# risc-mi/totalsegmentator2D

Measured on AMD Instinct MI355X. Metric: 2-ch 512x512 slices/sec, higher is better.
Workload: dtype f32 storage/accumulate, products as 3x fp16-split MFMA (f16x3)

## Files before the change

totalsegmentator2d_amd/_lib.py:

```python
from __future__ import annotations

import ctypes
import os

_HERE = os.path.dirname(os.path.abspath(__file__))
LIB_PATH = os.path.join(_HERE, 'libts2d_engine.so')
HEADER_PATH = os.path.join(os.path.dirname(_HERE), 'include', 'ts2d_engine.h')
ABI_VERSION = 9
MAX_STAGES = 16
PRECISION_F32_EXACT = 0
PRECISION_F32_SPLIT_F16X3 = 1
PRECISION_F16 = 2

class ArchDesc(ctypes.Structure):
    _fields_ = [('input_channels', ctypes.c_int32), ('num_classes', ctypes.c_int32), ('n_stages', ctypes.c_int32),
                ('features', ctypes.c_int32 * MAX_STAGES), ('n_conv_enc', ctypes.c_int32 * MAX_STAGES),
                ('n_conv_dec', ctypes.c_int32 * MAX_STAGES), ('norm_eps', ctypes.c_float), ('leaky_slope', ctypes.c_float),
                ('strides', (ctypes.c_int32 * 2) * MAX_STAGES)]


class ResidualDesc(ctypes.Structure):
    _fields_ = [('n_blocks', ctypes.c_int32 * MAX_STAGES), ('reserved', ctypes.c_int32 * 16)]


class TiledImage(ctypes.Structure):
    _fields_ = [('image', ctypes.c_void_p), ('Hp', ctypes.c_int32), ('Wp', ctypes.c_int32), ('n_tiles', ctypes.c_int32),
                ('tile_y', ctypes.c_void_p), ('tile_x', ctypes.c_void_p), ('logits_f16', ctypes.c_void_p), ('seg_u8', ctypes.c_void_p),
                ('inf_flag', ctypes.c_int32)]


class TiledExport(ctypes.Structure):
    _fields_ = [('src_y', ctypes.c_int32), ('src_x', ctypes.c_int32), ('src_h', ctypes.c_int32), ('src_w', ctypes.c_int32),
                ('out_h', ctypes.c_int32), ('out_w', ctypes.c_int32), ('seg_u8', ctypes.c_void_p), ('logits_f32', ctypes.c_void_p)]


class TiledLabelmap(ctypes.Structure):
    _fields_ = [('src_y', ctypes.c_int32), ('src_x', ctypes.c_int32), ('src_h', ctypes.c_int32), ('src_w', ctypes.c_int32),
                ('out_h', ctypes.c_int32), ('out_w', ctypes.c_int32), ('label_u8', ctypes.c_void_p)]


class TiledProbabilities(ctypes.Structure):
    _fields_ = [('src_y', ctypes.c_int32), ('src_x', ctypes.c_int32), ('src_h', ctypes.c_int32), ('src_w', ctypes.c_int32),
                ('out_h', ctypes.c_int32), ('out_w', ctypes.c_int32), ('full_h', ctypes.c_int32), ('full_w', ctypes.c_int32),
                ('box_y', ctypes.c_int32), ('box_x', ctypes.c_int32), ('prob_f32', ctypes.c_void_p), ('decided_u8', ctypes.c_void_p)]


PROB_MULTILABEL, PROB_LABELMAP, PROB_REGIONS = 0, 1, 2

_I, _P, _Z, _LL, _ULL, _S = ctypes.c_int, ctypes.c_void_p, ctypes.c_size_t, ctypes.c_longlong, ctypes.c_ulonglong, ctypes.c_char_p
_PP, _TI, _TE, _TL = ctypes.POINTER(_P), ctypes.POINTER(TiledImage), ctypes.POINTER(TiledExport), ctypes.POINTER(TiledLabelmap)
_TP = ctypes.POINTER(TiledProbabilities)
_PROJECT = [_I, _P, _Z, _I, _I, _I, _I, _LL, _LL, _LL, _LL, _P, _P]

SIGNATURES = {
    'ts2d_abi_version': (_I, []),
    'ts2d_last_error': (_S, []),
    'ts2d_engine_create': (_I, [ctypes.POINTER(ArchDesc), _P, _Z, _I, _PP]),
    'ts2d_engine_create_residual': (_I, [ctypes.POINTER(ArchDesc), ctypes.POINTER(ResidualDesc), _P, _Z, _I, _PP]),
    'ts2d_engine_load_weights': (_I, [_P, _P, _Z]),
# ... 9 lines not shown
    'ts2d_labelmap_from_logits': (_I, [_I, _P, _I, _I, _I, ctypes.POINTER(ctypes.c_int32 * 4), _I, _I, _P]),
    'ts2d_ensemble_predict_tiled_regions': (_I, [_PP, _I, _TI, _TL, _I, _I, _I, _I, _P, _I, _P, _I]),
    'ts2d_regions_from_logits': (_I, [_I, _P, _I, _I, _I, ctypes.POINTER(ctypes.c_int32 * 4), _I, _I, _P, _P]),
    'ts2d_ensemble_predict_tiled_probabilities': (_I, [_PP, _I, _TI, _TP, _I, _I, _I, _I, _P, _I, _I, _P, _I]),
    'ts2d_probabilities_from_logits': (_I, [_I, _P, _I, _I, _I, ctypes.POINTER(ctypes.c_int32 * 4), _I, _I, _I, _I, _I, _I, _I, _P, _P, _P]),
    'ts2d_project_coronal': (_I, _PROJECT),
    'ts2d_project_coronal_zscore': (_I, _PROJECT + [_P, _P, _P]),
    'ts2d_resample_cubic': (_I, [_I, _P, _I, _I, _I, _I, _I, _P, _P]),
    'ts2d_planes_create': (_I, [_I, _P, _I, _I, _I, _PP]),
    'ts2d_planes_crop_zscore': (_I, [_P, ctypes.POINTER(ctypes.c_int32 * 4), _P, ctypes.POINTER(_I)]),
    'ts2d_planes_crop_normalize': (_I, [_P, _P, _P, _P, ctypes.POINTER(ctypes.c_int32 * 4), _P, ctypes.POINTER(_I)]),
    'ts2d_planes_create_stack': (_I, [_I, _P, _I, _I, _I, _I, _PP]),
    'ts2d_planes_crop_normalize_stack': (_I, [_P, _P, _P, _P, ctypes.POINTER(ctypes.c_int32 * 6), _P, ctypes.POINTER(_I)]),
    'ts2d_planes_resample_cubic': (_I, [_P, _I, _I]),
    'ts2d_planes_extent': (_I, [_P, ctypes.POINTER(_I), ctypes.POINTER(_I)]),
    'ts2d_planes_download': (_I, [_P, _P]),
    'ts2d_planes_destroy': (_I, [_P]),
    'ts2d_synth_slices': (_I, [_I, _ULL, _ULL, _ULL, _P, _P]),
    'ts2d_engine_reserve': (_I, [_P, _I, _I, _I]),
    'ts2d_engine_workspace_bytes': (_I, [_P, _I, _I, _I, ctypes.POINTER(_Z)]),
    'ts2d_engine_set_workspace': (_I, [_P, _P, _Z]),
    'ts2d_engine_set_precision': (_I, [_P, _I]),
    'ts2d_engine_set_option': (_I, [_P, _S, _I]),
    'ts2d_engine_set_tile_dtype': (_I, [_P, _I]),
    'ts2d_engine_set_keep_activations': (_I, [_P, _I]),
    'ts2d_engine_set_profiling': (_I, [_P, _I]),
    'ts2d_engine_num_ops': (_I, [_P]),
    'ts2d_engine_op_name': (_S, [_P, _I]),
    'ts2d_engine_op_kernel': (_S, [_P, _I]),
    'ts2d_engine_op_ksplit': (_I, [_P, _I]),
    'ts2d_engine_op_times': (_I, [_P, _P, _I]),
    'ts2d_engine_debug_tensor': (_I, [_P, _S, _P, _Z, ctypes.POINTER(ctypes.c_int32 * 4)]),
    'ts2d_engine_tiled_inf_flag': (_I, [_P]),
    'ts2d_engine_device_bytes': (_Z, [_P]),
    'ts2d_engine_destroy': (_I, [_P]),
}
SYMBOLS = tuple(SIGNATURES)
OPTIONAL = frozenset(n for n in SIGNATURES if n == 'ts2d_resample_cubic' or n.startswith('ts2d_planes_') or 'probabilities' in n or n == 'ts2d_engine_create_residual')


class EngineLibraryError(RuntimeError):
    pass


_lib = None


def build(verbose: bool = False) -> str:
    import subprocess
    subprocess.check_call(['make', '-C', os.path.join(_HERE, 'csrc')] + ([] if verbose else ['-s']))
    return LIB_PATH


def load():
    global _lib
    if _lib is not None:
        return _lib
    if not os.path.exists(LIB_PATH):
        raise EngineLibraryError(
            f"{LIB_PATH} is missing: the MI355X HIP engine has not been built (run `python -c 'import "
            f"__graft_entry__ as g; g.build()'` or `make -C totalsegmentator2d_amd/csrc`). There is no CPU fallback.")
    try:
        lib = ctypes.CDLL(LIB_PATH)
    except OSError as ex:
        raise EngineLibraryError(f"failed to load {LIB_PATH}: {ex}") from ex
    for name, (restype, argtypes) in SIGNATURES.items():
        if name in OPTIONAL and not hasattr(lib, name):
            continue
        fn = getattr(lib, name)
        fn.restype, fn.argtypes = restype, list(argtypes)
        if name == 'ts2d_abi_version' and fn() != ABI_VERSION:
            raise EngineLibraryError(f"ABI mismatch: library {fn()}, binding {ABI_VERSION}")
    _lib = lib
    return lib


def load_cffi():
    try:
        import cffi
    except ImportError:
        return None
    import re
    ffi = cffi.FFI()
    src = open(HEADER_PATH).read()
    src = re.sub(r'/\*.*?\*/', '', src, flags=re.S)
    src = '\n'.join(l for l in src.splitlines() if not l.strip().startswith('#') and 'extern "C"' not in l
                    and l.strip() not in ('}',))
    src = src.replace('TS2D_MAX_STAGES', str(MAX_STAGES))
    ffi.cdef(src)
    return ffi, ffi.dlopen(LIB_PATH)


def last_error() -> str:
    return load().ts2d_last_error().decode('utf-8', 'replace')


def check(rc: int, what: str):
    if rc != 0:
        raise RuntimeError(f"{what} failed ({rc}): {last_error()}")
```

totalsegmentator2d_amd/csrc/engine.hip:

```cpp
#include "engine_internal.h"
#include "kernels.h"
#include "kernels_f16x3.h"
#include "kernels_f16x3_convt.h"
#include "kernels_h32.h"
#include "kernels_head.h"
#include "kernels_f16x3_one.h"
#include "kernels_f16x3_qp.h"
#include "kernels_first.h"
#include "kernels_res32.h"
#include "kernels_s2v2.h"
#include "kernels_upc.h"
#include "kernels_up0.h"
#include "kernels_upq.h"
#include "kernels_upc_h.h"
#include "kernels_upc_h2.h"
#include "kernels_resblock.h"

#include <atomic>
#include <cstdio>
#include <cmath>
#include <cstdlib>
#include <cstring>
#include <string>
#include <type_traits>
// ... 611 lines not shown
    TRY(workspace_acquire(e, st));
    if (e->ws_external) {
        e->ws_token = ++g_ws_generation;
        if (!e->ws_token) e->ws_token = ++g_ws_generation;
        HIP_TRY(hipMemsetD32Async(reinterpret_cast<hipDeviceptr_t>(e->d_ws), (int)e->ws_token, 1, st));
    }
    if (clear_flags) HIP_TRY(hipMemsetAsync(e->d_flags, 0, 2 * sizeof(int), st));
    const int rc = run_forward_impl(e, d_in, B, H, W, d_logits, d_mask, st, full);
    const int rc2 = workspace_release(e, st);
    return rc != TS2D_OK ? rc : rc2;
}

int ts2d::reserve_checked(ts2d_engine* e, int B, int H, int W, bool full) {
    const int divy = 1 << e->lvl_y[e->arch.n_stages - 1], divx = 1 << e->lvl_x[e->arch.n_stages - 1];
    if (B < 1 || H < divy || W < divx || H % divy || W % divx)
        return fail(TS2D_ERR_INVALID, "shape B=%d H=%d W=%d: H and W must be positive multiples of %d and %d", B, H, W, divy, divx);
    if ((H / divy) * (W / divx) <= 1)
        return fail(TS2D_ERR_INVALID, "shape %dx%d leaves a single bottleneck pixel: InstanceNorm needs more than 1 spatial element", H, W);
    if ((long long)B * H * W >= (1LL << 31)) return fail(TS2D_ERR_INVALID, "B*H*W = %lld exceeds 2^31 pixels per call", (long long)B * H * W);
    return ensure_workspace(e, B, H, W, full);
}

extern "C" {

int ts2d_abi_version(void) { return 9; }

const char* ts2d_last_error(void) { return last_error(); }

static int create_engine(const char* entry, const ts2d_arch_desc* arch, const ts2d_residual_desc* res, const float* weights, size_t n_floats, int device,
                         ts2d_engine** out) {
    if (!arch || !out) return fail(TS2D_ERR_INVALID, "%s: null argument", entry);
    *out = nullptr;
    if (res) for (int v : res->reserved) if (v) return fail(TS2D_ERR_INVALID, "%s: ts2d_residual_desc.reserved must be zero", entry);
    int ndev = 0;
    HIP_TRY(hipGetDeviceCount(&ndev));
    if (device < 0 || device >= ndev) return fail(TS2D_ERR_INVALID, "device %d out of range (%d HIP devices visible)", device, ndev);
    ts2d_engine* e = new (std::nothrow) ts2d_engine();
    if (!e) return fail(TS2D_ERR_NOMEM, "host allocation failed");
    e->user_arch = *arch; e->device = device;
    if (res) { e->residual = true; for (int s = 0; s < TS2D_MAX_STAGES; ++s) e->n_blocks[s] = res->n_blocks[s]; }
    if (arch->n_stages >= 2 && arch->n_stages <= TS2D_MAX_STAGES) e->arch = pad_arch(*arch, e->padded); else e->arch = *arch;
    {
        hipDeviceProp_t prop;
        if (hipGetDeviceProperties(&prop, device) == hipSuccess && prop.multiProcessorCount > 0) e->num_cus = prop.multiProcessorCount;
        if (getenv("TS2D_DBG")) e->dbg = atoi(getenv("TS2D_DBG"));
    }
    int rc = build_program(e);
    if (rc != TS2D_OK) { delete e; return rc; }
    hipError_t he = hipSetDevice(device);
    if (he == hipSuccess) he = hipStreamCreateWithFlags(&e->stream, hipStreamNonBlocking);
    if (he == hipSuccess) he = hipEventCreateWithFlags(&e->ws_event, hipEventDisableTiming);
    if (he == hipSuccess) he = hipMalloc(reinterpret_cast<void**>(&e->d_flags), 2 * sizeof(int));
    if (he == hipSuccess) he = hipMemset(e->d_flags, 0, 2 * sizeof(int));
    if (he == hipSuccess && e->dbg == 256) he = hipMalloc(reinterpret_cast<void**>(&e->d_prof), 512 * 128 * sizeof(unsigned long long));
    if (he == hipSuccess && e->d_prof) he = hipMemset(e->d_prof, 0, 512 * 128 * sizeof(unsigned long long));
    if (he == hipSuccess) he = hipMalloc(reinterpret_cast<void**>(&e->d_weights), e->weight_floats * sizeof(float));
    if (he != hipSuccess) {
        rc = fail(he == hipErrorOutOfMemory ? TS2D_ERR_NOMEM : TS2D_ERR_HIP, "engine setup failed: %s", hipGetErrorString(he));
        ts2d_engine_destroy(e);
        return rc;
    }
    if (weights) {
        rc = upload_weights(e, weights, n_floats);
        if (rc != TS2D_OK) { ts2d_engine_destroy(e); return rc; }
    }
    *out = e;
    return TS2D_OK;
}

int ts2d_engine_create(const ts2d_arch_desc* arch, const float* weights, size_t n_floats, int device, ts2d_engine** out) {
    return create_engine("ts2d_engine_create", arch, nullptr, weights, n_floats, device, out);
}

int ts2d_engine_create_residual(const ts2d_arch_desc* arch, const ts2d_residual_desc* residual, const float* weights, size_t n_floats, int device,
                                ts2d_engine** out) {
    if (!residual) return fail(TS2D_ERR_INVALID, "ts2d_engine_create_residual: null argument");
    return create_engine("ts2d_engine_create_residual", arch, residual, weights, n_floats, device, out);
}

int ts2d_engine_load_weights(ts2d_engine* e, const float* weights, size_t n_floats) {
    if (!e || !weights) return fail(TS2D_ERR_INVALID, "ts2d_engine_load_weights: null argument");
    HIP_TRY(hipSetDevice(e->device));
    if (e->ws_busy) { HIP_TRY(hipEventSynchronize(e->ws_event)); e->ws_busy = false; }
    HIP_TRY(hipStreamSynchronize(e->stream));
    return upload_weights(e, weights, n_floats);
}

int ts2d_engine_weight_buffer(ts2d_engine* e, void** dev_ptr, size_t* n_bytes) {
    if (!e || !dev_ptr || !n_bytes) return fail(TS2D_ERR_INVALID, "ts2d_engine_weight_buffer: null argument");
    *dev_ptr = e->d_weights; *n_bytes = e->weight_floats * sizeof(float);
    return TS2D_OK;
}

int ts2d_engine_set_precision(ts2d_engine* e, int mode) {
    if (!e) return fail(TS2D_ERR_INVALID, "ts2d_engine_set_precision: null engine");
    if (mode != TS2D_PRECISION_F32_EXACT && mode != TS2D_PRECISION_F32_SPLIT_F16X3 && mode != TS2D_PRECISION_F16)
        return fail(TS2D_ERR_INVALID, "unknown precision mode %d", mode);
    if (mode == TS2D_PRECISION_F16 && e->residual)
        return fail(TS2D_ERR_INVALID, "TS2D_PRECISION_F16 is not supported on a residual-encoder engine (TS2D_PRECISION_F32_SPLIT_F16X3 and "
                    "TS2D_PRECISION_F32_EXACT are); the mode is unchanged");
    e->precision = mode;
    return TS2D_OK;
}

int ts2d_engine_set_option(ts2d_engine* e, const char* name, int value) {
    if (!e || !name) return fail(TS2D_ERR_INVALID, "ts2d_engine_set_option: null argument");
    struct B { const char* n; bool* p; };
// ... 277 lines not shown
```

totalsegmentator2d_amd/csrc/kernels.h:

```cpp
#pragma once
#include <hip/hip_runtime.h>
#include <stdint.h>
#include "tile_dims.h"
#include "device_tables.h"

typedef float f32x4 __attribute__((ext_vector_type(4)));
typedef float f32x16 __attribute__((ext_vector_type(16)));

namespace ts2d {

__device__ __forceinline__ void lds_barrier() { asm volatile("s_waitcnt lgkmcnt(0)\n\ts_barrier" ::: "memory"); }

constexpr f32x16 kZero16 = {0.f, 0.f, 0.f, 0.f, 0.f, 0.f, 0.f, 0.f, 0.f, 0.f, 0.f, 0.f, 0.f, 0.f, 0.f, 0.f};

#define TS2D_PROF_DECL(PROF) long long tacc_[7] = {0, 0, 0, 0, 0, 0, 0}, tlast_ = (PROF) ? (long long)__builtin_readcyclecounter() : 0
#define TS2D_STAMP_AT(PROF, I) if (PROF) { const long long t_ = (long long)__builtin_readcyclecounter(); tacc_[I] += t_ - tlast_; tlast_ = t_; }
#define TS2D_PROF_FLUSH(PROF) if ((PROF) && threadIdx.x == 0) {        \
        unsigned long long* p_ = (PROF) + (blockIdx.x & 63) * 8; \
        _Pragma("unroll") for (int i_ = 0; i_ < 7; ++i_) atomicAdd(p_ + i_, (unsigned long long)tacc_[i_]); \
        atomicAdd(p_ + 7, 1ull); }


__device__ __forceinline__ float stat_pivot(float v_first) { return __shfl(v_first, (int)(threadIdx.x & 31)); }
__device__ __forceinline__ void stat_wave_put(float* red, int slot, float s, float q, float kv, float n) {
    *reinterpret_cast<f32x4*>(red + 4 * slot) = f32x4{s, q, kv, n};
}
__device__ __forceinline__ void stat_tile_store(const float* red, int nwaves, int bn, int col, float* part_entry) {
    f32x4 a = *reinterpret_cast<const f32x4*>(red + 4 * col);
    for (int ww = 1; ww < nwaves; ++ww) {
        const f32x4 b = *reinterpret_cast<const f32x4*>(red + 4 * (ww * bn + col));
        const float d = b[2] - a[2];
        a[1] += b[1] + d * (2.f * b[0] + b[3] * d);
        a[0] += b[0] + b[3] * d;
        a[3] += b[3];
    }
    *reinterpret_cast<f32x4*>(part_entry) = a;
}

#if defined(__HIP_DEVICE_COMPILE__)
#define TS2D_PACKED_F32 __attribute__((target("packed-fp32-ops")))
#else
#define TS2D_PACKED_F32
#endif


__device__ __forceinline__ int fdiv(int n, float inv_d) { return (int)(((float)n + 0.5f) * inv_d); }
__device__ __forceinline__ int udiv_magic(int n, unsigned mg) { return mg ? (int)__umulhi((unsigned)n, mg) : n; }

struct ConvArgs {
    const float* src0; const float* sc0; const float* sh0; int C0;
    const float* src1; const float* sc1; const float* sh1; int C1;
    const float* wp;
    const float* bias;
    float* dst;
    float* part;
    int B, Hin, Win;
    int Ht, Wt;
    int N;
    int Cout;
    int TH, TW, NIMG;
    float inv_tw, inv_thw;
    int lgTH, lgTW;
    int tiles_x, tiles_y;
    int n_mtiles, n_ctiles;
    unsigned mg_tx, mg_tpi;
    int PH, PW;
    int KA, KB;
    float slope;
    const void* wph;
    int ksplit;
    long long kslice_stride;
    unsigned long long* prof;
    int dbg;
// ... 470 lines not shown
```

totalsegmentator2d_amd/csrc/kernels_s2v2.h:

```cpp
#pragma once
#include "kernels_f16x3.h"
#include "kernels_h32.h"

namespace ts2d {

constexpr int kS2Threads = 512;
constexpr int kS2PW = 66, kS2Slots = 17 * kS2PW;
constexpr int kS2Plane = (kS2Slots + 2) * 16;
static_assert(kS2Plane % 128 == 64, "plane stride of conv3x3s2_v2");

template <int BN, typename ST, int NP, bool RESW, bool FLEX = false, bool K32 = false>
__global__ __launch_bounds__(kS2Threads, 2) void conv3x3s2_v2(const ConvArgs a) {
    static_assert(!K32 || (NP == 1 && sizeof(ST) == 2), "32-channel chunks: fp16 storage, one product");
    constexpr int NPP = NP == 3 ? 2 : 1;
    constexpr int PARTS = K32 ? 2 : NPP;
    constexpr int CK = K32 ? 32 : 16;
    constexpr int NTW = BN / 64;
    constexpr int WTAP = PARTS * 2 * BN * 16, WB = 9 * WTAP;
    constexpr bool F32 = sizeof(ST) == 4;
    constexpr bool Q4 = F32 || K32;
    constexpr int MAXU = Q4 ? 9 : 5;
    constexpr int USTEP = Q4 ? 128 : 256;
    constexpr int DEPTH = BN == 64 ? 2 : 1;
    extern __shared__ __attribute__((aligned(16))) unsigned char smem8[];
    typedef unsigned u32x4 __attribute__((ext_vector_type(4)));
    typedef __attribute__((address_space(3))) void* lds_ptr;
    const int TH = FLEX ? a.TH : 8, TW = FLEX ? a.TW : 32;
    const int PW2 = FLEX ? 2 * TW + 2 : kS2PW, HO = FLEX ? TW + 1 : 33, PSL = FLEX ? (2 * TH + 1) * PW2 : kS2Slots;

    const int xcd = blockIdx.x & 7, q80 = blockIdx.x >> 3;
    const int qm0 = q80 / a.n_ctiles;
    const int ctile = q80 - qm0 * a.n_ctiles, n0col = ctile * BN;
    const int mtile0 = qm0 * 8 + xcd, mstep = ((int)(gridDim.x >> 3) / a.n_ctiles) * 8;
    if (mtile0 >= a.n_mtiles) return;
    const int ntl = (a.n_mtiles - 1 - mtile0) / mstep + 1;
    const int nchunks = a.C0 / CK;
    const int tpi = a.tiles_x * a.tiles_y;

    const int tid = threadIdx.x, lane = tid & 63;
    const int w = __builtin_amdgcn_readfirstlane(tid >> 6), wm = w & 3, wn = w >> 2;
    const int r = lane & 31, h = lane >> 5;

    unsigned char* sA = smem8;
    unsigned char* sB = smem8 + PARTS * 2 * kS2Plane;

    const int sub = Q4 ? (tid & 3) : ((lane >> 3) & 1);
    const int slot0 = Q4 ? (tid >> 2) : (32 * w + (lane & 7) + 8 * (lane >> 4));
    unsigned rel[MAXU];
    unsigned emask = 0;
    const int lw0 = F32 ? (sub >> 1) * kS2Plane + slot0 * 16 + (sub & 1) * 8 : sub * kS2Plane + slot0 * 16;
#pragma unroll
    for (int it = 0; it < MAXU; ++it) {
        const int q = slot0 + USTEP * it;
        const int py = q / PW2, rem = q - py * PW2;
        const int half = rem >= HO ? 1 : 0, px = 2 * (rem - HO * half) + half;
        const bool exists = q < PSL && px <= 2 * TW;
        rel[it] = exists ? (unsigned)(((py * a.Win + px) * a.C0) * (int)sizeof(ST) + 16 * sub) : 0x80000000u;
        if (exists) emask |= ((py == 0 ? 1u : 0u) | (px == 0 ? 2u : 0u)) << (2 * it);
        if (q < PSL && !exists) {
            if constexpr (F32) {
                *reinterpret_cast<uint2*>(sA + lw0 + it * USTEP * 16) = uint2{0u, 0u};
                if (NPP == 2) *reinterpret_cast<uint2*>(sA + lw0 + it * USTEP * 16 + 2 * kS2Plane) = uint2{0u, 0u};
            } else {
                *reinterpret_cast<uint4*>(sA + lw0 + it * USTEP * 16) = uint4{0u, 0u, 0u, 0u};
            }
        }
    }
    if constexpr (RESW) {
        constexpr int WIT = (WB / 16 + kS2Threads - 1) / kS2Threads;
        for (int c = 0; c < nchunks; ++c) {
            const uint4* wsrc = reinterpret_cast<const uint4*>(reinterpret_cast<const unsigned char*>(a.wph) + ((size_t)(K32 ? 2 * c : c) * a.n_ctiles + ctile) * (9 * 2 * 2 * BN * 16));
            constexpr int C16 = 9 * 4 * BN;
#pragma unroll
            for (int k = 0; k < WIT; ++k) {
                const int sl = tid + k * kS2Threads;
                if (WB / 16 % kS2Threads == 0 || sl < WB / 16) {
                    int src = sl;
                    if constexpr (K32) src = ((sl / (2 * BN)) & 1) * (C16 * a.n_ctiles) + (sl / (4 * BN)) * (4 * BN) + sl % (2 * BN);
                    else if constexpr (NPP == 1) src = (sl / (2 * BN)) * (4 * BN) + sl % (2 * BN);
                    *reinterpret_cast<uint4*>(sB + c * WB + sl * 16) = wsrc[src];
                }
            }
        }
    }

    struct Item { int k, c; };
    auto advance = [&](Item& t) {
        int c = t.c + 1, k = t.k;
        if (c == nchunks) { c = 0; ++k; }
        if (k < ntl) { t.k = k; t.c = c; }
    };
    auto tile_origin = [&](int k, int& nimg, int& tyi, int& txi, int& tin) {
        const int mtile = mtile0 + k * mstep;
        nimg = udiv_magic(mtile, a.mg_tpi); tin = mtile - nimg * tpi;
        tyi = udiv_magic(tin, a.mg_tx); txi = tin - tyi * a.tiles_x;
    };
    const size_t img_px = (size_t)a.Hin * a.Win;
    struct Stage { u32x4 pv[MAXU]; f32x4 nsa, nsb, nta, ntb; };
    Stage sg0, sg1;
    const bool normed = a.sc0 != nullptr;
    auto load_norm = [&](Stage& S, int nimg, int c) {
        const int co = F32 ? 4 * sub : 8 * sub;
        const float* ps = (normed ? a.sc0 : a.bias) + (normed ? (size_t)nimg * a.C0 + c * CK + co : 0);
        const float* pt = (normed ? a.sh0 : a.bias) + (normed ? (size_t)nimg * a.C0 + c * CK + co : 0);
        S.nsa = *reinterpret_cast<const f32x4*>(ps); S.nta = *reinterpret_cast<const f32x4*>(pt);
        if constexpr (!F32) { S.nsb = *reinterpret_cast<const f32x4*>(ps + 4); S.ntb = *reinterpret_cast<const f32x4*>(pt + 4); }
    };
    struct Req { __amdgpu_buffer_rsrc_t rs; unsigned org; int soff; };
    auto request = [&](const Item& t, int& nimg) {
        int tyi, txi, tin;
        tile_origin(t.k, nimg, tyi, txi, tin);
        Req q;
        q.rs = __builtin_amdgcn_make_buffer_rsrc(const_cast<ST*>(reinterpret_cast<const ST*>(a.src0)) + (size_t)nimg * img_px * a.C0, 0,
                                                 (int)(img_px * a.C0 * sizeof(ST)), 0x00020000);
        q.org = FLEX ? (unsigned)((((2 * TH * tyi - 1) * a.Win + 2 * TW * txi - 1) * a.C0) * (int)sizeof(ST))
                     : (unsigned)((((16 * tyi - 1) * a.Win + 64 * txi - 1) * a.C0) * (int)sizeof(ST));
        q.soff = t.c * CK * (int)sizeof(ST);
        return q;
    };
    auto load_unit = [&](Stage& S, const Req& q, int it) {
        const unsigned vo = rel[it] == 0x80000000u ? 0x80000000u : q.org + rel[it];
        S.pv[it] = __builtin_amdgcn_raw_buffer_load_b128(q.rs, vo, q.soff, 0);
    };

    Item cur{0, 0}, pf{0, 0};
    {
        int nimg;
        const Req q = request(cur, nimg);
#pragma unroll
        for (int it = 0; it < MAXU; ++it) load_unit(sg0, q, it);
        load_norm(sg0, nimg, cur.c);
        if constexpr (DEPTH == 2) {
            advance(pf);
            const Req q1 = request(pf, nimg);
#pragma unroll
            for (int it = 0; it < MAXU; ++it) load_unit(sg1, q1, it);
            load_norm(sg1, nimg, pf.c);
        }
    }

    const int abase = h * kS2Plane + ((4 * wm) * kS2PW + r) * 16;
    int fxb[2] = {0, 0};
    if constexpr (FLEX) {
#pragma unroll
        for (int mt = 0; mt < 2; ++mt) {
            const int m = 64 * wm + 32 * mt + r;
            const int ty = fdiv(m, a.inv_tw), tx = m - ty * TW;
            fxb[mt] = h * kS2Plane + (m < TH * TW ? (2 * ty * PW2 + tx) * 16 : 0);
        }
    }
    const int bbase = PARTS * 2 * kS2Plane + h * BN * 16 + (wn * (BN / 2) + r) * 16;
    const _Float16 slope_h = (_Float16)a.slope;
    const unsigned slope2 = (unsigned)__builtin_bit_cast(unsigned short, slope_h) * 0x10001u;
    const f32x4 slope4 = f32x4{a.slope, a.slope, a.slope, a.slope};

    f32x16 acc_t[2][NTW];
#pragma unroll
    for (int mt = 0; mt < 2; ++mt)
#pragma unroll
        for (int nt = 0; nt < NTW; ++nt)
#pragma unroll
            for (int i = 0; i < 16; ++i) acc_t[mt][nt][i] = 0.f;

    TS2D_PROF_DECL(a.prof);
    const int nitems = ntl * nchunks;
    const bool younger = w >= 4 && !(a.dbg & 512);
    auto item = [&](Stage& S) {
        int nimg0, tyi, txi, tin;
        tile_origin(cur.k, nimg0, tyi, txi, tin);
        const int ty0 = tyi * TH, tx0 = txi * TW;
        TS2D_STAMP_AT(a.prof, 3)
        lds_barrier();
        TS2D_STAMP_AT(a.prof, 1)
        const f32x4 nsa = S.nsa, nsb = S.nsb, nta = S.nta, ntb = S.ntb;
        if constexpr (!RESW) {
#pragma unroll
            for (int it = 0; it < MAXU; ++it) asm volatile("" :: "v"(S.pv[it]));
            asm volatile("" :: "v"(nsa), "v"(nta));
            if constexpr (!F32) asm volatile("" :: "v"(nsb), "v"(ntb));
            TS2D_STAMP_AT(a.prof, 2)
            const unsigned char* wsrc = reinterpret_cast<const unsigned char*>(a.wph) + ((size_t)(K32 ? 2 * cur.c : cur.c) * a.n_ctiles + ctile) * (9 * 2 * 2 * BN * 16) + lane * 16;
            constexpr int NPIECE = WB / 1024, RUN = 2 * BN * 16 / 1024;
            const size_t c16 = (size_t)a.n_ctiles * (9 * 2 * 2 * BN * 16);
#pragma unroll
            for (int j = 0; j < (NPIECE + 7) / 8; ++j) {
                const int pc = w + 8 * j;
                if (NPIECE % 8 == 0 || pc < NPIECE) {
                    size_t so;
                    if constexpr (K32) so = (size_t)((pc / RUN) & 1) * c16 + (size_t)((pc / (2 * RUN)) * 2 * RUN + pc % RUN) * 1024;
                    else so = (size_t)(NPP == 2 ? pc : (pc / RUN) * 2 * RUN + pc % RUN) * 1024;
                    __builtin_amdgcn_global_load_lds(wsrc + so, (lds_ptr)(sB + pc * 1024), 16, 0, 0);
                }
            }
        }
        constexpr unsigned kRow0 = Q4 ? 0x15555u : 0x155u, kCol0 = Q4 ? 0x2AAAAu : 0x2AAu;
        const unsigned pad = (tyi == 0 ? kRow0 : 0u) | (txi == 0 ? kCol0 : 0u);
        const bool border = pad != 0u;
#pragma unroll
        for (int it = 0; it < MAXU; ++it) {
            if (rel[it] != 0x80000000u) {
                unsigned char* d = sA + lw0 + it * USTEP * 16;
                const bool real = ((emask & pad) >> (2 * it) & 3u) == 0u;
                if constexpr (F32) {
                    f32x4 va = __builtin_bit_cast(f32x4, S.pv[it]);
                    if (normed) {
                        va = va * nsa + nta;
                        const f32x4 na = va * slope4;
#pragma unroll
                        for (int e = 0; e < 4; ++e) va[e] = fmaxf(va[e], na[e]);
                    }
                    uint2 hi, lo;
                    split_hi_lo_4(va, hi, lo);
                    if (border) { hi.x = real ? hi.x : 0u; hi.y = real ? hi.y : 0u; lo.x = real ? lo.x : 0u; lo.y = real ? lo.y : 0u; }
                    *reinterpret_cast<uint2*>(d) = hi;
                    if (NPP == 2) *reinterpret_cast<uint2*>(d + 2 * kS2Plane) = lo;
                } else {
                    uint4 x = uint4{S.pv[it][0], S.pv[it][1], S.pv[it][2], S.pv[it][3]};
                    if (normed) x = norm_lrelu_8(x, nsa, nsb, nta, ntb, slope2);
                    if (border) { x.x = real ? x.x : 0u; x.y = real ? x.y : 0u; x.z = real ? x.z : 0u; x.w = real ? x.w : 0u; }
                    *reinterpret_cast<uint4*>(d) = x;
                }
            }
        }
        TS2D_STAMP_AT(a.prof, 6)
        if constexpr (!RESW) asm volatile("s_waitcnt vmcnt(0)" ::: "memory");
        lds_barrier();
        TS2D_STAMP_AT(a.prof, 0)
        advance(pf);
        int nimg_pf;
        const Req rq = request(pf, nimg_pf);
        f32x16 acc_c[K32 ? 1 : 2][K32 ? 1 : NTW];
        const unsigned char* pw = smem8 + bbase + (RESW ? cur.c * WB : 0);
        __builtin_amdgcn_s_setprio(1);
        auto load_frags = [&](half8 (&fa)[2][PARTS], half8 (&fb)[NTW][PARTS], int tap) {
            const int dy = tap / 3, dx = tap - 3 * dy;
            const int toff = (dy * PW2 + (dx & 1) * HO + (dx >> 1)) * 16;
#pragma unroll
            for (int mt = 0; mt < 2; ++mt)
#pragma unroll
                for (int p = 0; p < PARTS; ++p)
                    fa[mt][p] = *reinterpret_cast<const half8*>(smem8 + (FLEX ? fxb[mt] : abase + mt * 2 * kS2PW * 16) + p * 2 * kS2Plane + toff);
#pragma unroll
            for (int nt = 0; nt < NTW; ++nt)
#pragma unroll
                for (int p = 0; p < PARTS; ++p) fb[nt][p] = *reinterpret_cast<const half8*>(pw + tap * WTAP + p * 2 * BN * 16 + nt * 512);
        };
        auto mma = [&](half8 (&fa)[2][PARTS], half8 (&fb)[NTW][PARTS], bool first) {
            if constexpr (K32) {
#pragma unroll
                for (int p = 0; p < 2; ++p)
#pragma unroll
                    for (int mt = 0; mt < 2; ++mt)
#pragma unroll
                        for (int nt = 0; nt < NTW; ++nt) acc_t[mt][nt] = __builtin_amdgcn_mfma_f32_32x32x16_f16(fa[mt][p], fb[nt][p], acc_t[mt][nt], 0, 0, 0);
            } else if constexpr (NP == 3) {
#pragma unroll
                for (int mt = 0; mt < 2; ++mt)
#pragma unroll
                    for (int nt = 0; nt < NTW; ++nt) acc_c[mt][nt] = __builtin_amdgcn_mfma_f32_32x32x16_f16(fa[mt][1], fb[nt][0], first ? kZero16 : acc_c[mt][nt], 0, 0, 0);
#pragma unroll
                for (int mt = 0; mt < 2; ++mt)
#pragma unroll
                    for (int nt = 0; nt < NTW; ++nt) acc_c[mt][nt] = __builtin_amdgcn_mfma_f32_32x32x16_f16(fa[mt][0], fb[nt][1], acc_c[mt][nt], 0, 0, 0);
#pragma unroll
                for (int mt = 0; mt < 2; ++mt)
#pragma unroll
                    for (int nt = 0; nt < NTW; ++nt) acc_c[mt][nt] = __builtin_amdgcn_mfma_f32_32x32x16_f16(fa[mt][0], fb[nt][0], acc_c[mt][nt], 0, 0, 0);
            } else {
#pragma unroll
                for (int mt = 0; mt < 2; ++mt)
#pragma unroll
                    for (int nt = 0; nt < NTW; ++nt) acc_c[mt][nt] = __builtin_amdgcn_mfma_f32_32x32x16_f16(fa[mt][0], fb[nt][0], first ? kZero16 : acc_c[mt][nt], 0, 0, 0);
            }
        };
        {
            half8 fa0[2][PARTS], fb0[NTW][PARTS], fa1[2][PARTS], fb1[NTW][PARTS];
            load_frags(fa0, fb0, 0);
#define TS2D_TAP2(T) { if constexpr ((T) + 1 < 9) { if constexpr ((T) & 1) load_frags(fa0, fb0, (T) + 1); else load_frags(fa1, fb1, (T) + 1); } \
                if constexpr ((T) & 1) mma(fa1, fb1, false); else mma(fa0, fb0, (T) == 0); \
                if constexpr ((T) < MAXU) load_unit(S, rq, (T)); \
                __builtin_amdgcn_sched_barrier(0); }
            TS2D_TAP2(0) TS2D_TAP2(1) TS2D_TAP2(2) TS2D_TAP2(3) TS2D_TAP2(4) TS2D_TAP2(5) TS2D_TAP2(6) TS2D_TAP2(7) TS2D_TAP2(8)
#undef TS2D_TAP2
        }
        load_norm(S, nimg_pf, pf.c);
        __builtin_amdgcn_s_setprio(0);
        if (younger) __builtin_amdgcn_s_setprio(1);
        TS2D_STAMP_AT(a.prof, 5)
        if constexpr (!K32) {
#pragma unroll
            for (int mt = 0; mt < 2; ++mt)
#pragma unroll
                for (int nt = 0; nt < NTW; ++nt) acc_t[mt][nt] += acc_c[mt][nt];
        }

        if (cur.c == nchunks - 1) {
            const float oscale = *a.oscale;
            const size_t img_el = (size_t)a.Ht * a.Wt * a.Cout;
            const auto rsd = __builtin_amdgcn_make_buffer_rsrc(reinterpret_cast<ST*>(a.dst) + (size_t)nimg0 * img_el, 0, (int)(img_el * sizeof(ST)), 0x00020000);
            float st_s[NTW], st_q[NTW], st_k[NTW];
            float nvalid = 64.f;
            float bvs[NTW];
#pragma unroll
            for (int nt = 0; nt < NTW; ++nt) bvs[nt] = a.bias[n0col + wn * (BN / 2) + nt * 32 + r];
            if constexpr (FLEX) {
                const int thw = TH * TW;
#pragma unroll
                for (int nt = 0; nt < NTW; ++nt) {
                    st_k[nt] = stat_pivot(round_act<ST>(__builtin_fmaf(acc_t[0][nt][0], oscale, bvs[nt])));
                    st_s[nt] = 0.f; st_q[nt] = 0.f;
                }
                int cnt = 0;
#pragma unroll
                for (int mt = 0; mt < 2; ++mt)
#pragma unroll
                    for (int j = 0; j < 4; ++j) {
                        int m0 = 64 * wm + 32 * mt + 4 * h + 8 * j;
                        asm volatile("" : "+v"(m0));
                        const int ty = fdiv(m0, a.inv_tw), tx = m0 - ty * TW;
                        const bool ok = m0 < thw;
                        const unsigned vrun = ok ? (unsigned)((((ty0 + ty) * a.Wt + tx0 + tx) * a.Cout + n0col + wn * (BN / 2) + r) * (int)sizeof(ST)) : 0x80000000u;
                        cnt += ok ? 4 : 0;
#pragma unroll
                        for (int e4 = 0; e4 < 4; ++e4)
#pragma unroll
                            for (int nt = 0; nt < NTW; ++nt) {
                                const int i2 = 4 * j + e4;
                                float v = __builtin_fmaf(acc_t[mt][nt][i2], oscale, bvs[nt]);
                                buffer_store_act<ST>(v, rsd, vrun, (unsigned)((e4 * a.Cout + nt * 32) * (int)sizeof(ST)));
                                const float d = ok ? round_act<ST>(v) - st_k[nt] : 0.f;
                                st_s[nt] += d; st_q[nt] = __builtin_fmaf(d, d, st_q[nt]);
                                acc_t[mt][nt][i2] = 0.f;
                            }
                        __builtin_amdgcn_sched_barrier(0);
                    }
                cnt += __shfl_xor(cnt, 32);
                nvalid = (float)cnt;
            } else {
#pragma unroll
            for (int nt = 0; nt < NTW; ++nt) {
                const int co = n0col + wn * (BN / 2) + nt * 32 + r;
                const float bv = bvs[nt];
                const float kv = stat_pivot(round_act<ST>(__builtin_fmaf(acc_t[0][nt][0], oscale, bv)));
                float s = 0.f, q = 0.f;
#pragma unroll
                for (int mt = 0; mt < 2; ++mt) {
                    const int oy = ty0 + 2 * wm + mt, ox = tx0 + 4 * h;
                    const unsigned voff = (unsigned)(((oy * a.Wt + ox) * a.Cout + co) * (int)sizeof(ST));
#pragma unroll
                    for (int i2 = 0; i2 < 16; ++i2) {
                        const unsigned soff = (unsigned)((((i2 & 3) + 8 * (i2 >> 2)) * a.Cout) * (int)sizeof(ST));
                        float v = __builtin_fmaf(acc_t[mt][nt][i2], oscale, bv);
                        buffer_store_act<ST>(v, rsd, voff, soff);
                        const float d = round_act<ST>(v) - kv;
                        s += d; q = __builtin_fmaf(d, d, q);
                        acc_t[mt][nt][i2] = 0.f;
                    }
                }
                st_s[nt] = s; st_q[nt] = q; st_k[nt] = kv;
            }
            }
            TS2D_STAMP_AT(a.prof, 4)
            lds_barrier();
            float* red = reinterpret_cast<float*>(smem8);
#pragma unroll
            for (int nt = 0; nt < NTW; ++nt) {
                float s = st_s[nt], q = st_q[nt];
                s += __shfl_xor(s, 32); q += __shfl_xor(q, 32);
                if (h == 0) stat_wave_put(red, wm * BN + wn * (BN / 2) + nt * 32 + r, s, q, st_k[nt], nvalid);
            }
            lds_barrier();
            if (tid < BN) stat_tile_store(red, 4, BN, tid, a.part + ((size_t)(nimg0 * tpi + tin) * a.Cout + n0col + tid) * 4);
        }
        advance(cur);
    };
    for (int i = 0; i < nitems; i += DEPTH) {
        item(sg0);
        if constexpr (DEPTH == 2) { if (i + 1 < nitems) item(sg1); }
    }
    TS2D_PROF_FLUSH(a.prof)
}

}
```

Measured before the change: 2935.

## Compile out profiling stamps and cut register pressure in stride-2 conv kernel

Profiling stamp macros now compile to nothing unless the library is built with TS2D_STAMPS, and a separate stamps library is loaded when TS2D_DBG=256. The stride-2 conv kernel re-reads tile arguments from the kernarg segment on demand instead of keeping them live, recomputes the load request and border pad only when the tile changes, and folds the out-of-range mask into emask. The border and norm branches of the convert step are specialised at compile time via templated lambdas. Together these aim to free registers and drop per-item scalar work, at the cost of more code paths and extra scalar kernarg loads.

```diff
diff --git a/totalsegmentator2d_amd/_lib.py b/totalsegmentator2d_amd/_lib.py
--- a/totalsegmentator2d_amd/_lib.py
+++ b/totalsegmentator2d_amd/_lib.py
@@ -5,6 +5,8 @@
 
 _HERE = os.path.dirname(os.path.abspath(__file__))
 LIB_PATH = os.path.join(_HERE, 'libts2d_engine.so')
+STAMPS_LIB_PATH = os.path.join(_HERE, 'libts2d_engine_stamps.so')
+_DEFAULT_LIB_PATH = LIB_PATH
 HEADER_PATH = os.path.join(os.path.dirname(_HERE), 'include', 'ts2d_engine.h')
 ABI_VERSION = 9
 MAX_STAGES = 16
@@ -120,18 +122,25 @@
     return LIB_PATH
 
 
+def library_path() -> str:
+    if os.environ.get('TS2D_DBG', '').strip() == '256' and LIB_PATH == _DEFAULT_LIB_PATH and os.path.exists(STAMPS_LIB_PATH):
+        return STAMPS_LIB_PATH
+    return LIB_PATH
+
+
 def load():
     global _lib
     if _lib is not None:
         return _lib
-    if not os.path.exists(LIB_PATH):
+    path = library_path()
+    if not os.path.exists(path):
         raise EngineLibraryError(
-            f"{LIB_PATH} is missing: the MI355X HIP engine has not been built (run `python -c 'import "
+            f"{path} is missing: the MI355X HIP engine has not been built (run `python -c 'import "
             f"__graft_entry__ as g; g.build()'` or `make -C totalsegmentator2d_amd/csrc`). There is no CPU fallback.")
     try:
-        lib = ctypes.CDLL(LIB_PATH)
+        lib = ctypes.CDLL(path)
     except OSError as ex:
-        raise EngineLibraryError(f"failed to load {LIB_PATH}: {ex}") from ex
+        raise EngineLibraryError(f"failed to load {path}: {ex}") from ex
     for name, (restype, argtypes) in SIGNATURES.items():
         if name in OPTIONAL and not hasattr(lib, name):
             continue
diff --git a/totalsegmentator2d_amd/csrc/engine.hip b/totalsegmentator2d_amd/csrc/engine.hip
--- a/totalsegmentator2d_amd/csrc/engine.hip
+++ b/totalsegmentator2d_amd/csrc/engine.hip
@@ -687,7 +687,15 @@
     if (he == hipSuccess) he = hipEventCreateWithFlags(&e->ws_event, hipEventDisableTiming);
     if (he == hipSuccess) he = hipMalloc(reinterpret_cast<void**>(&e->d_flags), 2 * sizeof(int));
     if (he == hipSuccess) he = hipMemset(e->d_flags, 0, 2 * sizeof(int));
+#if defined(TS2D_STAMPS)
     if (he == hipSuccess && e->dbg == 256) he = hipMalloc(reinterpret_cast<void**>(&e->d_prof), 512 * 128 * sizeof(unsigned long long));
+#else
+    if (e->dbg == 256) {
+        static std::atomic<bool> told{false};
+        if (!told.exchange(true)) fprintf(stderr, "ts2d: TS2D_DBG=256 asks for in-kernel phase stamps, but this library was built without them "
+                                                  "(make STAMPS=1 builds libts2d_engine_stamps.so): no [phases] lines\n");
+    }
+#endif
     if (he == hipSuccess && e->d_prof) he = hipMemset(e->d_prof, 0, 512 * 128 * sizeof(unsigned long long));
     if (he == hipSuccess) he = hipMalloc(reinterpret_cast<void**>(&e->d_weights), e->weight_floats * sizeof(float));
     if (he != hipSuccess) {
diff --git a/totalsegmentator2d_amd/csrc/kernels.h b/totalsegmentator2d_amd/csrc/kernels.h
--- a/totalsegmentator2d_amd/csrc/kernels.h
+++ b/totalsegmentator2d_amd/csrc/kernels.h
@@ -13,12 +13,18 @@
 
 constexpr f32x16 kZero16 = {0.f, 0.f, 0.f, 0.f, 0.f, 0.f, 0.f, 0.f, 0.f, 0.f, 0.f, 0.f, 0.f, 0.f, 0.f, 0.f};
 
+#if defined(TS2D_STAMPS)
 #define TS2D_PROF_DECL(PROF) long long tacc_[7] = {0, 0, 0, 0, 0, 0, 0}, tlast_ = (PROF) ? (long long)__builtin_readcyclecounter() : 0
 #define TS2D_STAMP_AT(PROF, I) if (PROF) { const long long t_ = (long long)__builtin_readcyclecounter(); tacc_[I] += t_ - tlast_; tlast_ = t_; }
 #define TS2D_PROF_FLUSH(PROF) if ((PROF) && threadIdx.x == 0) {        \
         unsigned long long* p_ = (PROF) + (blockIdx.x & 63) * 8; \
         _Pragma("unroll") for (int i_ = 0; i_ < 7; ++i_) atomicAdd(p_ + i_, (unsigned long long)tacc_[i_]); \
         atomicAdd(p_ + 7, 1ull); }
+#else
+#define TS2D_PROF_DECL(PROF) do {} while (0)
+#define TS2D_STAMP_AT(PROF, I)
+#define TS2D_PROF_FLUSH(PROF)
+#endif
 
 
 __device__ __forceinline__ float stat_pivot(float v_first) { return __shfl(v_first, (int)(threadIdx.x & 31)); }
diff --git a/totalsegmentator2d_amd/csrc/kernels_s2v2.h b/totalsegmentator2d_amd/csrc/kernels_s2v2.h
--- a/totalsegmentator2d_amd/csrc/kernels_s2v2.h
+++ b/totalsegmentator2d_amd/csrc/kernels_s2v2.h
@@ -1,6 +1,7 @@
 #pragma once
 #include "kernels_f16x3.h"
 #include "kernels_h32.h"
+#include <type_traits>
 
 namespace ts2d {
 
@@ -35,7 +36,6 @@
     if (mtile0 >= a.n_mtiles) return;
     const int ntl = (a.n_mtiles - 1 - mtile0) / mstep + 1;
     const int nchunks = a.C0 / CK;
-    const int tpi = a.tiles_x * a.tiles_y;
 
     const int tid = threadIdx.x, lane = tid & 63;
     const int w = __builtin_amdgcn_readfirstlane(tid >> 6), wm = w & 3, wn = w >> 2;
@@ -49,6 +49,8 @@
     unsigned rel[MAXU];
     unsigned emask = 0;
     const int lw0 = F32 ? (sub >> 1) * kS2Plane + slot0 * 16 + (sub & 1) * 8 : sub * kS2Plane + slot0 * 16;
+    static_assert((MAXU - 1) * USTEP <= kS2Slots && kS2Plane == (kS2Slots + 2) * 16, "units before the last stay inside the plane");
+    const int lwl = slot0 + USTEP * (MAXU - 1) < kS2Slots + 2 ? lw0 + (MAXU - 1) * USTEP * 16 : lw0 + (kS2Slots + (slot0 & 1) - slot0) * 16;
 #pragma unroll
     for (int it = 0; it < MAXU; ++it) {
         const int q = slot0 + USTEP * it;
@@ -57,6 +59,7 @@
         const bool exists = q < PSL && px <= 2 * TW;
         rel[it] = exists ? (unsigned)(((py * a.Win + px) * a.C0) * (int)sizeof(ST) + 16 * sub) : 0x80000000u;
         if (exists) emask |= ((py == 0 ? 1u : 0u) | (px == 0 ? 2u : 0u)) << (2 * it);
+        else emask |= 1u << (18 + it);
         if (q < PSL && !exists) {
             if constexpr (F32) {
                 *reinterpret_cast<uint2*>(sA + lw0 + it * USTEP * 16) = uint2{0u, 0u};
@@ -88,14 +91,21 @@
     auto advance = [&](Item& t) {
         int c = t.c + 1, k = t.k;
         if (c == nchunks) { c = 0; ++k; }
+        const bool moved = k < ntl && k != t.k;
         if (k < ntl) { t.k = k; t.c = c; }
-    };
-    auto tile_origin = [&](int k, int& nimg, int& tyi, int& txi, int& tin) {
-        const int mtile = mtile0 + k * mstep;
-        nimg = udiv_magic(mtile, a.mg_tpi); tin = mtile - nimg * tpi;
-        tyi = udiv_magic(tin, a.mg_tx); txi = tin - tyi * a.tiles_x;
-    };
-    const size_t img_px = (size_t)a.Hin * a.Win;
+        return moved;
+    };
+    typedef const ConvArgs __attribute__((address_space(4)))* kernarg_ptr;
+    auto tile_args = [&]() {
+        kernarg_ptr p = (kernarg_ptr)(uintptr_t)__builtin_amdgcn_kernarg_segment_ptr();
+        asm volatile("" : "+s"(p));
+        return p;
+    };
+    auto tile_origin = [&](kernarg_ptr ta, int k, int& nimg, int& tyi, int& txi, int& tin) {
+        const int mtile = mtile0 + k * mstep, tx = ta->tiles_x;
+        nimg = udiv_magic(mtile, ta->mg_tpi); tin = mtile - nimg * (tx * ta->tiles_y);
+        tyi = udiv_magic(tin, ta->mg_tx); txi = tin - tyi * tx;
+    };
     struct Stage { u32x4 pv[MAXU]; f32x4 nsa, nsb, nta, ntb; };
     Stage sg0, sg1;
     const bool normed = a.sc0 != nullptr;
@@ -106,36 +116,44 @@
         S.nsa = *reinterpret_cast<const f32x4*>(ps); S.nta = *reinterpret_cast<const f32x4*>(pt);
         if constexpr (!F32) { S.nsb = *reinterpret_cast<const f32x4*>(ps + 4); S.ntb = *reinterpret_cast<const f32x4*>(pt + 4); }
     };
-    struct Req { __amdgpu_buffer_rsrc_t rs; unsigned org; int soff; };
-    auto request = [&](const Item& t, int& nimg) {
-        int tyi, txi, tin;
-        tile_origin(t.k, nimg, tyi, txi, tin);
+    struct Req { __amdgpu_buffer_rsrc_t rs; unsigned org; int nimg; };
+    auto request = [&](int k) {
+        const kernarg_ptr ta = tile_args();
+        int nimg, tyi, txi, tin;
+        tile_origin(ta, k, nimg, tyi, txi, tin);
         Req q;
-        q.rs = __builtin_amdgcn_make_buffer_rsrc(const_cast<ST*>(reinterpret_cast<const ST*>(a.src0)) + (size_t)nimg * img_px * a.C0, 0,
-                                                 (int)(img_px * a.C0 * sizeof(ST)), 0x00020000);
-        q.org = FLEX ? (unsigned)((((2 * TH * tyi - 1) * a.Win + 2 * TW * txi - 1) * a.C0) * (int)sizeof(ST))
-                     : (unsigned)((((16 * tyi - 1) * a.Win + 64 * txi - 1) * a.C0) * (int)sizeof(ST));
-        q.soff = t.c * CK * (int)sizeof(ST);
+        q.nimg = nimg;
+        const int Win = ta->Win, C0 = ta->C0, TH = FLEX ? ta->TH : 8, TW = FLEX ? ta->TW : 32;
+        const size_t img_px = (size_t)ta->Hin * Win;
+        q.rs = __builtin_amdgcn_make_buffer_rsrc(const_cast<ST*>(reinterpret_cast<const ST*>(ta->src0)) + (size_t)nimg * img_px * C0, 0,
+                                                 (int)(img_px * C0 * sizeof(ST)), 0x00020000);
+        q.org = FLEX ? (unsigned)((((2 * TH * tyi - 1) * Win + 2 * TW * txi - 1) * C0) * (int)sizeof(ST))
+                     : (unsigned)((((16 * tyi - 1) * Win + 64 * txi - 1) * C0) * (int)sizeof(ST));
         return q;
     };
-    auto load_unit = [&](Stage& S, const Req& q, int it) {
-        const unsigned vo = rel[it] == 0x80000000u ? 0x80000000u : q.org + rel[it];
-        S.pv[it] = __builtin_amdgcn_raw_buffer_load_b128(q.rs, vo, q.soff, 0);
+    auto load_unit = [&](Stage& S, const Req& q, int c, int it) {
+        const unsigned vo = (q.org + rel[it]) | ((emask << (13 - it)) & 0x80000000u);
+        S.pv[it] = __builtin_amdgcn_raw_buffer_load_b128(q.rs, vo, c * CK * (int)sizeof(ST), 0);
+    };
+    constexpr unsigned kRow0 = Q4 ? 0x15555u : 0x155u, kCol0 = Q4 ? 0x2AAAAu : 0x2AAu;
+    auto tile_pad = [&](int k) {
+        int nimg, tyi, txi, tin;
+        tile_origin(tile_args(), k, nimg, tyi, txi, tin);
+        return (tyi == 0 ? kRow0 : 0u) | (txi == 0 ? kCol0 : 0u);
     };
 
     Item cur{0, 0}, pf{0, 0};
+    Req rq = request(0);
+    unsigned pad = tile_pad(0);
     {
-        int nimg;
-        const Req q = request(cur, nimg);
-#pragma unroll
-        for (int it = 0; it < MAXU; ++it) load_unit(sg0, q, it);
-        load_norm(sg0, nimg, cur.c);
+#pragma unroll
+        for (int it = 0; it < MAXU; ++it) load_unit(sg0, rq, 0, it);
+        load_norm(sg0, rq.nimg, 0);
         if constexpr (DEPTH == 2) {
-            advance(pf);
-            const Req q1 = request(pf, nimg);
-#pragma unroll
-            for (int it = 0; it < MAXU; ++it) load_unit(sg1, q1, it);
-            load_norm(sg1, nimg, pf.c);
+            if (advance(pf)) rq = request(pf.k);
+#pragma unroll
+            for (int it = 0; it < MAXU; ++it) load_unit(sg1, rq, pf.c, it);
+            load_norm(sg1, rq.nimg, pf.c);
         }
     }
 
@@ -164,11 +182,8 @@
 
     TS2D_PROF_DECL(a.prof);
     const int nitems = ntl * nchunks;
-    const bool younger = w >= 4 && !(a.dbg & 512);
+    const int prio_off = a.dbg & 512;
     auto item = [&](Stage& S) {
-        int nimg0, tyi, txi, tin;
-        tile_origin(cur.k, nimg0, tyi, txi, tin);
-        const int ty0 = tyi * TH, tx0 = txi * TW;
         TS2D_STAMP_AT(a.prof, 3)
         lds_barrier();
         TS2D_STAMP_AT(a.prof, 1)
@@ -179,31 +194,30 @@
             asm volatile("" :: "v"(nsa), "v"(nta));
             if constexpr (!F32) asm volatile("" :: "v"(nsb), "v"(ntb));
             TS2D_STAMP_AT(a.prof, 2)
-            const unsigned char* wsrc = reinterpret_cast<const unsigned char*>(a.wph) + ((size_t)(K32 ? 2 * cur.c : cur.c) * a.n_ctiles + ctile) * (9 * 2 * 2 * BN * 16) + lane * 16;
+            const unsigned char* wsrc = reinterpret_cast<const unsigned char*>(a.wph) + ((size_t)(K32 ? 2 * cur.c : cur.c) * a.n_ctiles + ctile) * (9 * 2 * 2 * BN * 16);
             constexpr int NPIECE = WB / 1024, RUN = 2 * BN * 16 / 1024;
-            const size_t c16 = (size_t)a.n_ctiles * (9 * 2 * 2 * BN * 16);
+            const unsigned c16 = (unsigned)a.n_ctiles * (9 * 2 * 2 * BN * 16);
 #pragma unroll
             for (int j = 0; j < (NPIECE + 7) / 8; ++j) {
                 const int pc = w + 8 * j;
                 if (NPIECE % 8 == 0 || pc < NPIECE) {
-                    size_t so;
-                    if constexpr (K32) so = (size_t)((pc / RUN) & 1) * c16 + (size_t)((pc / (2 * RUN)) * 2 * RUN + pc % RUN) * 1024;
-                    else so = (size_t)(NPP == 2 ? pc : (pc / RUN) * 2 * RUN + pc % RUN) * 1024;
+                    unsigned so;
+                    if constexpr (K32) so = (unsigned)((pc / RUN) & 1) * c16 + (unsigned)((pc / (2 * RUN)) * 2 * RUN + pc % RUN) * 1024u + lane * 16u;
+                    else if constexpr (NPP == 2) so = (unsigned)tid * 16u + j * 8192u;
+                    else so = (unsigned)((pc / RUN) * 2 * RUN + pc % RUN) * 1024u + lane * 16u;
                     __builtin_amdgcn_global_load_lds(wsrc + so, (lds_ptr)(sB + pc * 1024), 16, 0, 0);
                 }
             }
         }
-        constexpr unsigned kRow0 = Q4 ? 0x15555u : 0x155u, kCol0 = Q4 ? 0x2AAAAu : 0x2AAu;
-        const unsigned pad = (tyi == 0 ? kRow0 : 0u) | (txi == 0 ? kCol0 : 0u);
-        const bool border = pad != 0u;
-#pragma unroll
-        for (int it = 0; it < MAXU; ++it) {
-            if (rel[it] != 0x80000000u) {
-                unsigned char* d = sA + lw0 + it * USTEP * 16;
+        auto convert = [&](auto border_c, auto normed_c) {
+            constexpr bool BORDER = decltype(border_c)::value, NORMED = decltype(normed_c)::value;
+#pragma unroll
+            for (int it = 0; it < MAXU; ++it) {
+                unsigned char* d = sA + (it == MAXU - 1 ? lwl : lw0 + it * USTEP * 16);
                 const bool real = ((emask & pad) >> (2 * it) & 3u) == 0u;
                 if constexpr (F32) {
                     f32x4 va = __builtin_bit_cast(f32x4, S.pv[it]);
-                    if (normed) {
+                    if constexpr (NORMED) {
                         va = va * nsa + nta;
                         const f32x4 na = va * slope4;
 #pragma unroll
@@ -211,24 +225,24 @@
                     }
                     uint2 hi, lo;
                     split_hi_lo_4(va, hi, lo);
-                    if (border) { hi.x = real ? hi.x : 0u; hi.y = real ? hi.y : 0u; lo.x = real ? lo.x : 0u; lo.y = real ? lo.y : 0u; }
+                    if constexpr (BORDER) { hi.x = real ? hi.x : 0u; hi.y = real ? hi.y : 0u; lo.x = real ? lo.x : 0u; lo.y = real ? lo.y : 0u; }
                     *reinterpret_cast<uint2*>(d) = hi;
                     if (NPP == 2) *reinterpret_cast<uint2*>(d + 2 * kS2Plane) = lo;
                 } else {
                     uint4 x = uint4{S.pv[it][0], S.pv[it][1], S.pv[it][2], S.pv[it][3]};
-                    if (normed) x = norm_lrelu_8(x, nsa, nsb, nta, ntb, slope2);
-                    if (border) { x.x = real ? x.x : 0u; x.y = real ? x.y : 0u; x.z = real ? x.z : 0u; x.w = real ? x.w : 0u; }
+                    if constexpr (NORMED) x = norm_lrelu_8(x, nsa, nsb, nta, ntb, slope2);
+                    if constexpr (BORDER) { x.x = real ? x.x : 0u; x.y = real ? x.y : 0u; x.z = real ? x.z : 0u; x.w = real ? x.w : 0u; }
                     *reinterpret_cast<uint4*>(d) = x;
                 }
             }
-        }
+        };
+        if (pad != 0u) { if (normed) convert(std::true_type{}, std::true_type{}); else convert(std::true_type{}, std::false_type{}); }
+        else { if (normed) convert(std::false_type{}, std::true_type{}); else convert(std::false_type{}, std::false_type{}); }
         TS2D_STAMP_AT(a.prof, 6)
         if constexpr (!RESW) asm volatile("s_waitcnt vmcnt(0)" ::: "memory");
         lds_barrier();
         TS2D_STAMP_AT(a.prof, 0)
-        advance(pf);
-        int nimg_pf;
-        const Req rq = request(pf, nimg_pf);
+        if (advance(pf)) rq = request(pf.k);
         f32x16 acc_c[K32 ? 1 : 2][K32 ? 1 : NTW];
         const unsigned char* pw = smem8 + bbase + (RESW ? cur.c * WB : 0);
         __builtin_amdgcn_s_setprio(1);
@@ -278,14 +292,18 @@
             load_frags(fa0, fb0, 0);
 #define TS2D_TAP2(T) { if constexpr ((T) + 1 < 9) { if constexpr ((T) & 1) load_frags(fa0, fb0, (T) + 1); else load_frags(fa1, fb1, (T) + 1); } \
                 if constexpr ((T) & 1) mma(fa1, fb1, false); else mma(fa0, fb0, (T) == 0); \
-                if constexpr ((T) < MAXU) load_unit(S, rq, (T)); \
+                if constexpr ((T) < MAXU) load_unit(S, rq, pf.c, (T)); \
                 __builtin_amdgcn_sched_barrier(0); }
             TS2D_TAP2(0) TS2D_TAP2(1) TS2D_TAP2(2) TS2D_TAP2(3) TS2D_TAP2(4) TS2D_TAP2(5) TS2D_TAP2(6) TS2D_TAP2(7) TS2D_TAP2(8)
 #undef TS2D_TAP2
         }
-        load_norm(S, nimg_pf, pf.c);
+        load_norm(S, rq.nimg, pf.c);
         __builtin_amdgcn_s_setprio(0);
-        if (younger) __builtin_amdgcn_s_setprio(1);
+        {
+            int wv = w;
+            asm volatile("" : "+s"(wv));
+            if (wv >= 4 && !prio_off) __builtin_amdgcn_s_setprio(1);
+        }
         TS2D_STAMP_AT(a.prof, 5)
         if constexpr (!K32) {
 #pragma unroll
@@ -295,16 +313,22 @@
         }
 
         if (cur.c == nchunks - 1) {
-            const float oscale = *a.oscale;
-            const size_t img_el = (size_t)a.Ht * a.Wt * a.Cout;
-            const auto rsd = __builtin_amdgcn_make_buffer_rsrc(reinterpret_cast<ST*>(a.dst) + (size_t)nimg0 * img_el, 0, (int)(img_el * sizeof(ST)), 0x00020000);
+            const kernarg_ptr eap = tile_args();
+            const struct { const float* oscale; const float* bias; float* dst; float* part; int Ht, Wt, Cout, TH, TW; float inv_tw; }
+                ea{eap->oscale, eap->bias, eap->dst, eap->part, eap->Ht, eap->Wt, eap->Cout, FLEX ? eap->TH : 8, FLEX ? eap->TW : 32, eap->inv_tw};
+            int nimg0, tyi, txi, tin;
+            tile_origin(eap, cur.k, nimg0, tyi, txi, tin);
+            const int tpi = eap->tiles_x * eap->tiles_y, ty0 = tyi * ea.TH, tx0 = txi * ea.TW;
+            const float oscale = *ea.oscale;
+            const size_t img_el = (size_t)ea.Ht * ea.Wt * ea.Cout;
+            const auto rsd = __builtin_amdgcn_make_buffer_rsrc(reinterpret_cast<ST*>(ea.dst) + (size_t)nimg0 * img_el, 0, (int)(img_el * sizeof(ST)), 0x00020000);
             float st_s[NTW], st_q[NTW], st_k[NTW];
             float nvalid = 64.f;
             float bvs[NTW];
 #pragma unroll
-            for (int nt = 0; nt < NTW; ++nt) bvs[nt] = a.bias[n0col + wn * (BN / 2) + nt * 32 + r];
+            for (int nt = 0; nt < NTW; ++nt) bvs[nt] = ea.bias[n0col + wn * (BN / 2) + nt * 32 + r];
             if constexpr (FLEX) {
-                const int thw = TH * TW;
+                const int thw = ea.TH * ea.TW;
 #pragma unroll
                 for (int nt = 0; nt < NTW; ++nt) {
                     st_k[nt] = stat_pivot(round_act<ST>(__builtin_fmaf(acc_t[0][nt][0], oscale, bvs[nt])));
@@ -317,9 +341,9 @@
                     for (int j = 0; j < 4; ++j) {
                         int m0 = 64 * wm + 32 * mt + 4 * h + 8 * j;
                         asm volatile("" : "+v"(m0));
-                        const int ty = fdiv(m0, a.inv_tw), tx = m0 - ty * TW;
+                        const int ty = fdiv(m0, ea.inv_tw), tx = m0 - ty * ea.TW;
                         const bool ok = m0 < thw;
-                        const unsigned vrun = ok ? (unsigned)((((ty0 + ty) * a.Wt + tx0 + tx) * a.Cout + n0col + wn * (BN / 2) + r) * (int)sizeof(ST)) : 0x80000000u;
+                        const unsigned vrun = ok ? (unsigned)((((ty0 + ty) * ea.Wt + tx0 + tx) * ea.Cout + n0col + wn * (BN / 2) + r) * (int)sizeof(ST)) : 0x80000000u;
                         cnt += ok ? 4 : 0;
 #pragma unroll
                         for (int e4 = 0; e4 < 4; ++e4)
@@ -327,7 +351,7 @@
                             for (int nt = 0; nt < NTW; ++nt) {
                                 const int i2 = 4 * j + e4;
                                 float v = __builtin_fmaf(acc_t[mt][nt][i2], oscale, bvs[nt]);
-                                buffer_store_act<ST>(v, rsd, vrun, (unsigned)((e4 * a.Cout + nt * 32) * (int)sizeof(ST)));
+                                buffer_store_act<ST>(v, rsd, vrun, (unsigned)((e4 * ea.Cout + nt * 32) * (int)sizeof(ST)));
                                 const float d = ok ? round_act<ST>(v) - st_k[nt] : 0.f;
                                 st_s[nt] += d; st_q[nt] = __builtin_fmaf(d, d, st_q[nt]);
                                 acc_t[mt][nt][i2] = 0.f;
@@ -346,10 +370,10 @@
 #pragma unroll
                 for (int mt = 0; mt < 2; ++mt) {
                     const int oy = ty0 + 2 * wm + mt, ox = tx0 + 4 * h;
-                    const unsigned voff = (unsigned)(((oy * a.Wt + ox) * a.Cout + co) * (int)sizeof(ST));
+                    const unsigned voff = (unsigned)(((oy * ea.Wt + ox) * ea.Cout + co) * (int)sizeof(ST));
 #pragma unroll
                     for (int i2 = 0; i2 < 16; ++i2) {
-                        const unsigned soff = (unsigned)((((i2 & 3) + 8 * (i2 >> 2)) * a.Cout) * (int)sizeof(ST));
+                        const unsigned soff = (unsigned)((((i2 & 3) + 8 * (i2 >> 2)) * ea.Cout) * (int)sizeof(ST));
                         float v = __builtin_fmaf(acc_t[mt][nt][i2], oscale, bv);
                         buffer_store_act<ST>(v, rsd, voff, soff);
                         const float d = round_act<ST>(v) - kv;
@@ -370,9 +394,9 @@
                 if (h == 0) stat_wave_put(red, wm * BN + wn * (BN / 2) + nt * 32 + r, s, q, st_k[nt], nvalid);
             }
             lds_barrier();
-            if (tid < BN) stat_tile_store(red, 4, BN, tid, a.part + ((size_t)(nimg0 * tpi + tin) * a.Cout + n0col + tid) * 4);
-        }
-        advance(cur);
+            if (tid < BN) stat_tile_store(red, 4, BN, tid, ea.part + ((size_t)(nimg0 * tpi + tin) * ea.Cout + n0col + tid) * 4);
+        }
+        if (advance(cur)) pad = tile_pad(cur.k);
     };
     for (int i = 0; i < nitems; i += DEPTH) {
         item(sg0);
```

Result: no change. 2952, median of 6 (+0.6%).
